# apache/arrow-go

Hardware: AMD Instinct MI355X
Metric: GB/s processed per kernel (Sum/Add/Filter/Take) vs HBM roofline (higher is better)
Workload: dtype int64+f64

## Files before the change

### arrow_go_amd/csrc/ah_common.h

```cpp
#pragma once
#include <hip/hip_runtime.h>
#include <initializer_list>
#include <type_traits>
#include <stdarg.h>
#include <stdint.h>
#include <stddef.h>
#include <stdio.h>
#include <stdlib.h>
#include <string.h>
#include "../../include/arrowhip.h"

#define AH_EXPORT extern "C" __attribute__((visibility("default")))

struct ah_filter_cache {
  bool valid;
  const uint8_t *fdata, *fvalid;
  int64_t foff, n, ntiles;
  int null_sel, tile_rows;
  void* buf;
  size_t bytes;
  int64_t* super_off;
  int* tile_local;
  int64_t* total;
};

struct ah_ctx {
  int device;
  hipStream_t stream;
  hipStream_t copy_stream;
  bool owns_stream;
  hipEvent_t ev_copy;
  hipEvent_t ev_compute;
  hipEvent_t t0, t1;
  hipEvent_t* marks;
  int n_marks;
  void* scratch;
  size_t scratch_bytes;
  void* temp;
  size_t temp_bytes;
  void* pack;
  size_t pack_bytes;
  uint64_t* pinned;
  uint64_t* dscalars;
  int num_cu;
  int tune_nt;
  int tune_blocks_per_cu;
  int opt_take_binned, opt_take_window_log2, opt_take_gather_wg, opt_take_gather_load, opt_take_gather_lds;
  int opt_groupby_keys;
  int opt_groupby_partition;
  int opt_encode_partition;
  int opt_encode_part_slots;
  int opt_encode_byte_map;
  int opt_encode_early_look;
  int opt_encode_part_min;
  int opt_hash_direct;
  int opt_hash_sum_partition;
  int opt_sort_msd;
  int opt_scan_segment_log2;
  void* expr_cache;
  int capturing;
  ah_filter_cache fcache;
  int opt_scan_onepass;
  void* scan_recs;
  size_t scan_recs_bytes;
  unsigned scan_epoch;
  int opt_groupby_seed;
  int opt_groupby_reserve;
  int opt_groupby_lean;
  int opt_filter_cache;
  int take_clustered_hint;
  int opt_take_vec;
  bool take_hint_valid, take_hint_live;
  const void* take_hint_idx; int64_t take_hint_nidx; int take_hint_kind, take_hint_near, take_hint_uses, opt_take_hint_cache;
  unsigned long long take_hint_word;
  int opt_arith_xcd_map;
  int opt_groupby_scale_guess;
  int opt_encode_unperm2_group;
  int opt_encode_resolve_wgs;
  int opt_encode_dict_compact;
  int opt_encode_table_batch;
  int opt_encode_unperm_group;
  int opt_take_vec_nt;
  unsigned long long* mailbox;
  unsigned long long mailbox_seq;
  char err[512];
};

static inline unsigned ah_stream_grid(const ah_ctx* c, int64_t work_items, int default_bpc = 8) {
  int bpc = c->tune_blocks_per_cu > 0 ? c->tune_blocks_per_cu : default_bpc;
  int64_t cap = bpc > 0 ? (int64_t)c->num_cu * bpc : ((int64_t)1 << 30);
  int64_t g = work_items < cap ? work_items : cap;
  return (unsigned)(g < 1 ? 1 : g);
}

static inline int ah_fail(ah_ctx* ctx, int code, const char* fmt, ...) __attribute__((format(printf, 3, 4)));
static inline int ah_fail(ah_ctx* ctx, int code, const char* fmt, ...) {
  if (ctx) {
    va_list ap;
    va_start(ap, fmt);
    vsnprintf(ctx->err, sizeof(ctx->err), fmt, ap);
    va_end(ap);
  }
  return code;
}

#define AH_HIP(ctx, call)                                                              \
  do {                                                                                 \
    hipError_t e__ = (call);                                                           \
    if (e__ != hipSuccess)                                                             \
      return ah_fail((ctx), AH_EHIP, "%s failed: %s (%s:%d)", #call, hipGetErrorString(e__), \
                     __FILE__, __LINE__);                                              \
  } while (0)

#define AH_ENTER_KEEP(ctx)                                             \
  do {                                                                 \
    if (!(ctx)) return AH_EINVALID;                                    \
    (ctx)->err[0] = 0;                                                 \
    AH_HIP((ctx), hipSetDevice((ctx)->device));                        \
  } while (0)

#define AH_ENTER(ctx)                                                  \
  do {                                                                 \
    AH_ENTER_KEEP(ctx);                                                \
    (ctx)->fcache.valid = false;                                       \
    (ctx)->take_hint_valid = false;                                    \
  } while (0)

static inline bool ah_take_hint_overlaps(const ah_ctx* c, const void* p, size_t nbytes) {
  if (!c->take_hint_valid || !c->take_hint_idx) return false;
  const uintptr_t a = (uintptr_t)p, b = a + nbytes, lo = (uintptr_t)c->take_hint_idx, hi = lo + (size_t)c->take_hint_nidx * (size_t)(c->take_hint_kind / 2);
  return a < hi && lo < b;
}
static inline bool ah_fcache_overlaps(const ah_ctx* c, const void* p, size_t nbytes) {
  if (!c->fcache.valid) return false;
  const uintptr_t a = (uintptr_t)p, b = a + nbytes;
  const uintptr_t lo = (uintptr_t)(c->fcache.foff >> 3), hi = (uintptr_t)((c->fcache.foff + c->fcache.n + 7) >> 3);
  for (const uint8_t* bm : {c->fcache.fdata, c->fcache.fvalid})
    if (bm && a < (uintptr_t)bm + hi && (uintptr_t)bm + lo < b) return true;
// ... 276 lines not shown
```

### arrow_go_amd/csrc/ah_ctx.hip

```cpp
#include <chrono>
#include "ah_common.h"

static const char* kVersion = "arrowhip 0.1 (gfx950)";

AH_EXPORT const char* ah_version(void) { return kVersion; }

AH_EXPORT int ah_device_count(int* n_host) {
  int n = 0;
  hipError_t e = hipGetDeviceCount(&n);
  if (n_host) *n_host = (e == hipSuccess) ? n : 0;
  return e == hipSuccess ? AH_OK : AH_EHIP;
}

static int ctx_init_common(ah_ctx* c) {
  AH_HIP(c, hipStreamCreateWithFlags(&c->copy_stream, hipStreamNonBlocking));
  AH_HIP(c, hipEventCreateWithFlags(&c->ev_copy, hipEventDisableTiming));
  AH_HIP(c, hipEventCreateWithFlags(&c->ev_compute, hipEventDisableTiming));
  AH_HIP(c, hipEventCreate(&c->t0));
  AH_HIP(c, hipEventCreate(&c->t1));
  AH_HIP(c, hipHostMalloc((void**)&c->pinned, 64 * sizeof(uint64_t), hipHostMallocDefault));
  AH_HIP(c, hipMalloc((void**)&c->dscalars, (kDsScalars + kPopcountMaxPartials) * sizeof(uint64_t)));
  AH_HIP(c, hipMemset(c->dscalars, 0, (kDsScalars + kPopcountMaxPartials) * sizeof(uint64_t)));
  AH_HIP(c, hipHostMalloc((void**)&c->mailbox, 256, hipHostMallocCoherent | hipHostMallocMapped));
  memset(c->mailbox, 0, 256);
  hipDeviceProp_t prop;
  AH_HIP(c, hipGetDeviceProperties(&prop, c->device));
  c->num_cu = prop.multiProcessorCount > 0 ? prop.multiProcessorCount : 256;
  const char* e_nt = getenv("ARROWHIP_NT");
  c->tune_nt = e_nt ? atoi(e_nt) : 1;
  const char* e_bpc = getenv("ARROWHIP_BLOCKS_PER_CU");
  c->tune_blocks_per_cu = e_bpc ? atoi(e_bpc) : 0;
  auto env_int = [](const char* name, int dflt) { const char* e = getenv(name); return e ? atoi(e) : dflt; };
  c->opt_take_binned = env_int("ARROWHIP_TAKE_BINNED", 1);
  c->opt_take_window_log2 = env_int("ARROWHIP_TAKE_WINDOW_LOG2", 22);
  c->opt_take_gather_wg = env_int("ARROWHIP_TAKE_GATHER_WG_PER_CU", 8);
  c->opt_groupby_partition = env_int("ARROWHIP_GROUPBY_PARTITION", 1);
  c->opt_groupby_keys = env_int("ARROWHIP_GROUPBY_KEYS", 1280);
  c->opt_hash_direct = env_int("ARROWHIP_HASH_DIRECT", 2);
  c->opt_hash_sum_partition = env_int("ARROWHIP_HASH_PARTITION", 1);
  c->opt_encode_partition = env_int("ARROWHIP_ENCODE_PARTITION", 1);
  c->opt_encode_part_min = env_int("ARROWHIP_ENCODE_PART_MIN", 300000);
  c->opt_encode_early_look = env_int("ARROWHIP_ENCODE_EARLY_LOOK", 1);
  c->opt_encode_byte_map = env_int("ARROWHIP_ENCODE_BYTE_MAP", 1);
  c->opt_encode_part_slots = env_int("ARROWHIP_ENCODE_PART_SLOTS", 8192);
  c->opt_sort_msd = env_int("ARROWHIP_SORT_MSD", 1);
  c->opt_scan_segment_log2 = env_int("ARROWHIP_SCAN_SEGMENT_LOG2", 0);
  c->opt_take_gather_lds = env_int("ARROWHIP_TAKE_GATHER_LDS", 1);
  c->opt_take_vec_nt = env_int("ARROWHIP_TAKE_VEC_NT", 7);
  c->opt_encode_unperm_group = env_int("ARROWHIP_ENCODE_UNPERM_GROUP", 4);
  c->opt_encode_table_batch = env_int("ARROWHIP_ENCODE_TABLE_BATCH", 1);
  c->opt_encode_dict_compact = env_int("ARROWHIP_ENCODE_DICT_COMPACT", 1);
  c->opt_encode_resolve_wgs = env_int("ARROWHIP_ENCODE_RESOLVE_WGS", 1024);
  c->opt_encode_unperm2_group = env_int("ARROWHIP_ENCODE_UNPERM2_GROUP", 4);
  c->opt_groupby_scale_guess = env_int("ARROWHIP_GROUPBY_SCALE_GUESS", 1);
  c->opt_arith_xcd_map = env_int("ARROWHIP_ARITH_XCD_MAP", 0);
  c->opt_take_vec = env_int("ARROWHIP_TAKE_VEC", 1);
  c->opt_take_gather_load = env_int("ARROWHIP_TAKE_GATHER_LOAD", 0);
  return AH_OK;
}

static int ctx_create(int device_id, void* stream, bool borrow, ah_ctx** out) {
  if (!out) return AH_EINVALID;
  *out = nullptr;
  ah_ctx* c = (ah_ctx*)calloc(1, sizeof(ah_ctx));
  if (!c) return AH_EINVALID;
  c->device = device_id;
  hipError_t e = hipSetDevice(device_id);
  if (e != hipSuccess) { free(c); return AH_EHIP; }
  if (borrow) {
    c->stream = (hipStream_t)stream;
    c->owns_stream = false;
  } else {
    e = hipStreamCreateWithFlags(&c->stream, hipStreamNonBlocking);
    if (e != hipSuccess) { free(c); return AH_EHIP; }
    c->owns_stream = true;
  }
  int rc = ctx_init_common(c);
  if (rc != AH_OK) { fprintf(stderr, "arrowhip: ctx init failed: %s\n", c->err); free(c); return rc; }
  c->opt_filter_cache = c->owns_stream ? 1 : 0;
  c->opt_take_hint_cache = c->owns_stream ? 1 : 0;
  c->opt_groupby_lean = 1;
  c->opt_scan_onepass = 1;
  c->opt_groupby_seed = 1;
  c->opt_groupby_reserve = 1;
  *out = c;
  return AH_OK;
}

AH_EXPORT int ah_ctx_create(int device_id, ah_ctx** out) { return ctx_create(device_id, nullptr, false, out); }
AH_EXPORT int ah_ctx_create_on_stream(int device_id, void* hip_stream, ah_ctx** out) {
  return ctx_create(device_id, hip_stream, true, out);
}

AH_EXPORT void ah_ctx_destroy(ah_ctx* c) {
  if (!c) return;
  (void)hipSetDevice(c->device);
  (void)hipStreamSynchronize(c->stream);
  (void)hipStreamSynchronize(c->copy_stream);
  ah_expr_cache_free(c);
  if (c->scratch) (void)hipFree(c->scratch);
  if (c->pinned) (void)hipHostFree(c->pinned);
  if (c->dscalars) (void)hipFree(c->dscalars);
  if (c->mailbox) (void)hipHostFree(c->mailbox);
  if (c->fcache.buf) (void)hipFree(c->fcache.buf);
  if (c->scan_recs) (void)hipFree(c->scan_recs);
  if (c->temp) (void)hipFree(c->temp);
  if (c->pack) (void)hipFree(c->pack);
  (void)hipEventDestroy(c->ev_copy);
  (void)hipEventDestroy(c->ev_compute);
  (void)hipEventDestroy(c->t0);
  (void)hipEventDestroy(c->t1);
  for (int i = 0; i < c->n_marks; i++) if (c->marks[i]) (void)hipEventDestroy(c->marks[i]);
  free(c->marks);
  (void)hipStreamDestroy(c->copy_stream);
  if (c->owns_stream) (void)hipStreamDestroy(c->stream);
  free(c);
}

AH_EXPORT int ah_ctx_set_option(ah_ctx* c, const char* name, int64_t value) {
  AH_ENTER(c);
  if (!name) return ah_fail(c, AH_EINVALID, "set_option: null name");
  if (!strcmp(name, "nt")) c->tune_nt = (int)value;
  else if (!strcmp(name, "blocks_per_cu")) c->tune_blocks_per_cu = (int)value;
  else if (!strcmp(name, "take_binned")) c->opt_take_binned = (int)value;
  else if (!strcmp(name, "take_window_log2")) c->opt_take_window_log2 = (int)value;
  else if (!strcmp(name, "take_gather_wg_per_cu")) c->opt_take_gather_wg = (int)value;
  else if (!strcmp(name, "take_gather_lds")) c->opt_take_gather_lds = (int)value;
  else if (!strcmp(name, "take_vec")) c->opt_take_vec = (int)value;
  else if (!strcmp(name, "take_hint_cache")) { c->opt_take_hint_cache = (int)value; c->take_hint_valid = false; }
  else if (!strcmp(name, "take_vec_nt")) c->opt_take_vec_nt = (int)value;
  else if (!strcmp(name, "encode_unperm_group")) c->opt_encode_unperm_group = (int)value;
  else if (!strcmp(name, "encode_table_batch")) c->opt_encode_table_batch = (int)value;
  else if (!strcmp(name, "encode_dict_compact")) c->opt_encode_dict_compact = (int)value;
  else if (!strcmp(name, "encode_unperm2_group")) c->opt_encode_unperm2_group = (int)value;
  else if (!strcmp(name, "encode_resolve_wgs")) c->opt_encode_resolve_wgs = value < 1 ? 1 : (int)value;
  else if (!strcmp(name, "groupby_scale_guess")) c->opt_groupby_scale_guess = (int)value;
  else if (!strcmp(name, "arith_xcd_map")) c->opt_arith_xcd_map = (int)value;
  else if (!strcmp(name, "take_gather_load")) c->opt_take_gather_load = (int)value;
  else if (!strcmp(name, "groupby_partition")) c->opt_groupby_partition = (int)value;
  else if (!strcmp(name, "groupby_keys")) c->opt_groupby_keys = (int)value;
  else if (!strcmp(name, "hash_direct")) c->opt_hash_direct = (int)value;
  else if (!strcmp(name, "hash_sum_partition")) c->opt_hash_sum_partition = (int)value;
  else if (!strcmp(name, "encode_partition")) c->opt_encode_partition = (int)value;
  else if (!strcmp(name, "encode_part_min")) c->opt_encode_part_min = (int)value;
  else if (!strcmp(name, "encode_early_look")) c->opt_encode_early_look = (int)value;
  else if (!strcmp(name, "encode_byte_map")) c->opt_encode_byte_map = (int)value;
  else if (!strcmp(name, "encode_part_slots")) c->opt_encode_part_slots = (int)value;
  else if (!strcmp(name, "sort_msd")) c->opt_sort_msd = (int)value;
  else if (!strcmp(name, "scan_onepass")) c->opt_scan_onepass = (int)value;
  else if (!strcmp(name, "groupby_lean")) c->opt_groupby_lean = (int)value;
  else if (!strcmp(name, "groupby_seed")) c->opt_groupby_seed = (int)value;
  else if (!strcmp(name, "groupby_reserve")) c->opt_groupby_reserve = (int)value;
  else if (!strcmp(name, "filter_cache")) { c->opt_filter_cache = value != 0; if (!value) c->fcache.valid = false; }
  else if (!strcmp(name, "scan_segment_log2")) c->opt_scan_segment_log2 = (int)value;
  else return ah_fail(c, AH_EINVALID, "set_option: unknown option '%s'", name);
  return AH_OK;
}

AH_EXPORT const char* ah_last_error(ah_ctx* c) { return c ? c->err : "null context"; }

namespace {
__global__ void mailbox_post_kernel(const unsigned long long* __restrict__ src, int nwords, const unsigned long long* __restrict__ src2, int nwords2,
                                    unsigned long long* mailbox, unsigned long long seq) {
  for (int i = 0; i < nwords; i++) __hip_atomic_store(&mailbox[i], src[i], __ATOMIC_RELAXED, __HIP_MEMORY_SCOPE_SYSTEM);
  for (int i = 0; i < nwords2; i++) __hip_atomic_store(&mailbox[nwords + i], src2[i], __ATOMIC_RELAXED, __HIP_MEMORY_SCOPE_SYSTEM);
  __hip_atomic_store(&mailbox[7], seq, __ATOMIC_RELEASE, __HIP_MEMORY_SCOPE_SYSTEM);
}
}
int ah_mailbox_read(ah_ctx* c, const unsigned long long* dev_words, int nwords, unsigned long long* out_host) {
  return ah_mailbox_read2(c, dev_words, nwords, nullptr, 0, out_host);
}
int ah_mailbox_begin(ah_ctx* c, unsigned long long** mb_out, unsigned long long* seq_out) {
  if (c->capturing) { c->capturing = 2; return ah_fail(c, AH_EINVALID, "this call returns a value to the host: it cannot be recorded into a graph"); }
  *mb_out = c->mailbox + 8;
  *seq_out = ++c->mailbox_seq;
  return AH_OK;
}
int ah_mailbox_wait(ah_ctx* c, unsigned long long seq, int nwords, unsigned long long* out_host) {
  if (nwords < 1 || nwords > 7) return ah_fail(c, AH_EINVALID, "mailbox_wait: 1..7 words");
  unsigned long long* mb = c->mailbox + 8;
  bool seen = false;
  const auto t0 = std::chrono::steady_clock::now();
  for (unsigned spin = 0;; spin++) {
    if (__atomic_load_n(&mb[7], __ATOMIC_ACQUIRE) == seq) { seen = true; break; }
    __builtin_ia32_pause();
    if ((spin & 1023u) == 1023u && std::chrono::steady_clock::now() - t0 > std::chrono::milliseconds(5)) break;
  }
  if (!seen) {
    AH_HIP(c, hipStreamSynchronize(c->stream));
    if (__atomic_load_n(&mb[7], __ATOMIC_ACQUIRE) != seq) return ah_fail(c, AH_EHIP, "mailbox_wait: the kernel did not report");
  }
  for (int i = 0; i < nwords; i++) out_host[i] = __atomic_load_n(&mb[i], __ATOMIC_RELAXED);
  return AH_OK;
}
int ah_mailbox_read2(ah_ctx* c, const unsigned long long* dev_words, int nwords, const unsigned long long* dev_words2, int nwords2,
                     unsigned long long* out_host) {
  if (nwords < 1 || nwords2 < 0 || nwords + nwords2 > 7) return ah_fail(c, AH_EINVALID, "mailbox_read: 1..7 words");
  if (c->capturing) { c->capturing = 2; return ah_fail(c, AH_EINVALID, "this call returns a value to the host: it cannot be recorded into a graph"); }
  unsigned long long* mb = c->mailbox + 8;
  const unsigned long long seq = ++c->mailbox_seq;
  mailbox_post_kernel<<<1, 1, 0, c->stream>>>(dev_words, nwords, dev_words2, nwords2, mb, seq);
  AH_LAUNCH_CHECK(c);
  bool seen = false;
  const auto t0 = std::chrono::steady_clock::now();
  for (unsigned spin = 0;; spin++) {
    if (__atomic_load_n(&mb[7], __ATOMIC_ACQUIRE) == seq) { seen = true; break; }
    __builtin_ia32_pause();
    if ((spin & 1023u) == 1023u && std::chrono::steady_clock::now() - t0 > std::chrono::milliseconds(5)) break;
  }
  if (!seen) {
    AH_HIP(c, hipStreamSynchronize(c->stream));
    if (__atomic_load_n(&mb[7], __ATOMIC_ACQUIRE) != seq) return ah_fail(c, AH_EHIP, "mailbox_read: the post kernel did not report");
  }
  for (int i = 0; i < nwords + nwords2; i++) out_host[i] = __atomic_load_n(&mb[i], __ATOMIC_RELAXED);
  return AH_OK;
}

int ah_scratch_reserve(ah_ctx* c, size_t nbytes, void** out) {
  if (nbytes > c->scratch_bytes) {
    AH_HIP(c, hipStreamSynchronize(c->stream));
    if (c->scratch) AH_HIP(c, hipFree(c->scratch));
    c->scratch = nullptr;
    c->scratch_bytes = 0;
    size_t want = (nbytes + ((size_t)1 << 20) - 1) & ~(((size_t)1 << 20) - 1);
// ... 295 lines not shown
```

### arrow_go_amd/csrc/ah_hash.hip

```cpp
#include "ah_common.h"
#include "ah_hashing.h"
#include "ah_bytes.h"

namespace {


struct Slot {
  unsigned long long key;
  unsigned first_row;
  unsigned id;
};


struct U64Keys {
  const unsigned long long* keys;
  static constexpr bool kLdsTable = true;
  __device__ __forceinline__ bool load(int64_t i, unsigned long long* word, uint64_t* h) const {
    const unsigned long long k = keys[i];
    *word = k;
    *h = hash_int(k);
    return k != kEmpty;
  }
  __device__ __forceinline__ bool same(unsigned long long cur, unsigned long long word, int64_t) const { return cur == word; }
};
// ... 137 lines not shown
      k[u] = 0;
      idx[u] = 0;
      if (i < hi) {
        if (ah_bit(valid, off + i)) {
          uint64_t h;
          if (!keys.load(i, &k[u], &h)) { kind[u] = 2; idx[u] = cap; }
          else { kind[u] = 1; idx[u] = h & mask; }
        } else if (encode_nulls) { kind[u] = 2; idx[u] = cap + 1; }
        else kind[u] = 3;
      }
    }
#pragma unroll
    for (int u = 0; u < kInsertRows; u++)
      if (kind[u] == 1 || kind[u] == 2) sv[u] = load_slot(&table[idx[u]]);
#pragma unroll
    for (int u = 0; u < kInsertRows; u++) {
      const int64_t i = base + (int64_t)u * kBlock;
      if (kind[u] == 0) continue;
      if (kind[u] == 3) { if (row_slot) row_slot[i] = direct_below ? 0u : kNoRow; continue; }
      uint64_t s = idx[u];
      unsigned fr = sv[u].first_row;
      unsigned id = sv[u].id;
      if (kind[u] == 1) {
        unsigned long long cur = sv[u].key;
        int probes = 0;
        for (;;) {
          if (cur == kEmpty) {
            cur = atomicCAS(&table[s].key, kEmpty, k[u]);
            if (cur == kEmpty) { fresh++; break; }
          }
          if (keys.same(cur, k[u], i)) break;
          s = (s + 1) & mask;
          if (++probes > kProbeLimit) { atomicExch(overflow, 1u); return; }
          const SlotView nx = load_slot(&table[s]);
          cur = nx.key;
          fr = nx.first_row;
          id = nx.id;
        }
      }
      if (fr < direct_below) {
        if (row_slot) row_slot[i] = id;
        continue;
      }
      if (fr > (unsigned)i) atomicMin(&table[s].first_row, (unsigned)i);
      if (row_slot) row_slot[i] = (unsigned)s | flag;
      nmiss++;
    }
  }
  if (fresh) atomicAdd(distinct, (unsigned long long)fresh);
  if (direct_below && nmiss) atomicAdd(misses, (unsigned long long)nmiss);
}

__global__ __launch_bounds__(kBlock) void mark_kernel(const Slot* __restrict__ table, uint64_t nslots,
                                                       unsigned long long* __restrict__ firsts) {
  const int64_t stride = (int64_t)gridDim.x * kBlock;
  for (uint64_t s = (uint64_t)blockIdx.x * kBlock + threadIdx.x; s < nslots; s += stride) {
    unsigned fr = table[s].first_row;
    if (fr != kNoRow) atomicOr(&firsts[fr >> 6], 1ull << (fr & 63));
  }
}


__global__ __launch_bounds__(kBlock) void assign_kernel(Slot* __restrict__ table, uint64_t cap, const unsigned long long* __restrict__ firsts,
                                                         const unsigned* __restrict__ wordprefix, const int64_t* __restrict__ tileoff,
                                                         unsigned long long* __restrict__ dict, int* __restrict__ null_id,
                                                         long long* __restrict__ first_rows) {
  const int64_t stride = (int64_t)gridDim.x * kBlock;
  const uint64_t nslots = cap + 2;
  for (uint64_t s = (uint64_t)blockIdx.x * kBlock + threadIdx.x; s < nslots; s += stride) {
    unsigned fr = table[s].first_row;
    if (fr == kNoRow) continue;
    unsigned id = rank_of_row(fr, firsts, wordprefix, tileoff);
    table[s].id = id;
    if (first_rows) first_rows[id] = (long long)fr;
    if (s == cap + 1) {
      *null_id = (int)id;
      if (dict) dict[id] = 0;
    } else if (dict) {
      dict[id] = table[s].key;
    }
  }
}

__global__ __launch_bounds__(kBlock) void emit_kernel(const Slot* __restrict__ table, int32_t* __restrict__ ids, int64_t n, int64_t direct_from) {
  constexpr int U = 4;
  const int64_t stride = (int64_t)gridDim.x * kBlock * U;
  for (int64_t base = (int64_t)blockIdx.x * kBlock * U + threadIdx.x; base < n; base += stride) {
    unsigned s[U];
    int32_t id[U];
    bool put[U];
#pragma unroll
    for (int u = 0; u < U; u++) {
      const int64_t i = base + (int64_t)u * kBlock;
      s[u] = i < n ? (unsigned)ids[i] : kNoRow;
      put[u] = i < n;
      if (i >= direct_from && s[u] != kNoRow) {
        if (s[u] & 0x80000000u) s[u] &= 0x7fffffffu; else put[u] = false;
      }
    }
#pragma unroll
    for (int u = 0; u < U; u++) id[u] = s[u] == kNoRow ? 0 : (put[u] ? (int32_t)table[s[u]].id : 0);
#pragma unroll
    for (int u = 0; u < U; u++) {
      const int64_t i = base + (int64_t)u * kBlock;
      if (put[u]) ids[i] = id[u];
    }
  }
}

constexpr unsigned kLookup = 0xFFFFFFFEu;
struct InsertSide {
  uint64_t cap;
  int encode_nulls;
  unsigned ones_id, null_id;
  __device__ __forceinline__ InsertSide(const Slot* t, uint64_t cap_, int encode_nulls_)
      : cap(cap_), encode_nulls(encode_nulls_), ones_id(t[cap_].first_row != kNoRow ? t[cap_].id : kNoRow),
        null_id(t[cap_ + 1].first_row != kNoRow ? t[cap_ + 1].id : kNoRow) {}
};

__device__ __forceinline__ bool claim_slot(unsigned long long k, Slot* __restrict__ table, uint64_t mask, int limit, unsigned* __restrict__ overflow,
                                           uint64_t* slot, unsigned* inserted) {
  uint64_t s = hash_int(k) & mask;
  int probes = 0;
  for (;;) {
    unsigned long long cur = table[s].key;
    if (cur != k && cur == kEmpty) {
      cur = atomicCAS(&table[s].key, kEmpty, k);
      if (cur == kEmpty) { (*inserted)++; cur = k; }
    }
    if (cur == k) break;
    s = (s + 1) & mask;
    if (++probes > limit) { atomicExch(overflow, 1u); return false; }
  }
  *slot = s;
  return true;
}

__device__ __forceinline__ unsigned row_without_lookup(const InsertSide& t, bool ok, unsigned long long k, uint64_t* s) {
  *s = ok ? t.cap : t.cap + 1;
  if (!ok) return t.encode_nulls ? t.null_id : 0u;
  return k == kEmpty ? t.ones_id : kLookup;
}
__device__ __forceinline__ bool miss_row(Slot* __restrict__ table, uint64_t mask, unsigned* __restrict__ overflow, unsigned long long k, int64_t i, bool probe,
                                         uint64_t s, unsigned* fresh, unsigned* nmiss, unsigned* r) {
  if (probe && !claim_slot(k, table, mask, kProbeLimit, overflow, &s, fresh)) return false;
  if (table[s].first_row > (unsigned)i) atomicMin(&table[s].first_row, (unsigned)i);
  *r = 0x80000000u | (unsigned)s;
  (*nmiss)++;
  return true;
}

constexpr int kSmallSlots = 8192;
constexpr int kSmallKeys = 4096;
constexpr int kSmallBlock = 1024;
constexpr int kSmallRows = 8;

__global__ __launch_bounds__(kBlock) void small_build_kernel(const Slot* __restrict__ table, uint64_t cap,
                                                              unsigned long long* __restrict__ skeys, unsigned* __restrict__ sids) {
  const int64_t stride = (int64_t)gridDim.x * kBlock;
  for (uint64_t s = (uint64_t)blockIdx.x * kBlock + threadIdx.x; s < cap; s += stride) {
    if (table[s].first_row == kNoRow) continue;
    const unsigned long long k = table[s].key;
    unsigned j = (unsigned)hash_int(k) & (kSmallSlots - 1);
    while (atomicCAS(&skeys[j], kEmpty, k) != kEmpty) j = (j + 1) & (kSmallSlots - 1);
    sids[j] = table[s].id;
  }
// ... 74 lines not shown
  unsigned long long key;
  unsigned id;
  unsigned pad;
};
__global__ __launch_bounds__(kBlock) void compact_build_kernel(const Slot* __restrict__ table, uint64_t cap, CSlot* __restrict__ ctab, uint64_t cmask) {
  const int64_t stride = (int64_t)gridDim.x * kBlock;
  for (uint64_t s = (uint64_t)blockIdx.x * kBlock + threadIdx.x; s < cap; s += stride) {
    const SlotView v = load_slot(&table[s]);
    if (v.first_row == kNoRow) continue;
    uint64_t j = hash_int(v.key) & cmask;
    while (atomicCAS(&ctab[j].key, kEmpty, v.key) != kEmpty) j = (j + 1) & cmask;
    ctab[j].id = v.id;
  }
}

constexpr int kCompactRows = 8;
__global__ __launch_bounds__(kBlock) void insert_compact_kernel(const unsigned long long* __restrict__ keys, const uint8_t* __restrict__ valid,
                                                                 int64_t off, int64_t lo, int64_t hi, int encode_nulls, Slot* __restrict__ table,
                                                                 uint64_t cap, const CSlot* __restrict__ ctab, uint64_t cmask,
                                                                 unsigned* __restrict__ out_ids, unsigned long long* __restrict__ distinct,
                                                                 unsigned* __restrict__ overflow, unsigned long long* __restrict__ misses) {
  const InsertSide side(table, cap, encode_nulls);
  const uint64_t mask = cap - 1;
  const int64_t stride = (int64_t)gridDim.x * kBlock * kCompactRows;
  unsigned fresh = 0, nmiss = 0;
  for (int64_t base = lo + (int64_t)blockIdx.x * kBlock * kCompactRows + threadIdx.x; base < hi; base += stride) {
    unsigned long long k[kCompactRows];
    bool ok[kCompactRows];
    uint4 cs[kCompactRows];
#pragma unroll
    for (int u = 0; u < kCompactRows; u++) {
      const int64_t i = base + (int64_t)u * kBlock;
      ok[u] = i < hi && ah_bit(valid, off + i);
      k[u] = ok[u] ? __builtin_nontemporal_load(&keys[i]) : 0ull;
    }
#pragma unroll
    for (int u = 0; u < kCompactRows; u++) cs[u] = *reinterpret_cast<const uint4*>(&ctab[hash_int(k[u]) & cmask]);
#pragma unroll
    for (int u = 0; u < kCompactRows; u++) {
      const int64_t i = base + (int64_t)u * kBlock;
      if (i >= hi) break;
      uint64_t s;
      bool probe = false;
      unsigned r = row_without_lookup(side, ok[u], k[u], &s);
      if (r == kLookup) {
        r = kNoRow;
        uint64_t j = hash_int(k[u]) & cmask;
        uint4 c = cs[u];
        for (;;) {
          const unsigned long long ck = ((unsigned long long)c.y << 32) | c.x;
          if (ck == k[u]) { r = c.z; break; }
          if (ck == kEmpty) { probe = true; break; }
          j = (j + 1) & cmask;
          c = *reinterpret_cast<const uint4*>(&ctab[j]);
        }
      }
      if (r == kNoRow && !miss_row(table, mask, overflow, k[u], i, probe, s, &fresh, &nmiss, &r)) return;
      if (out_ids) __builtin_nontemporal_store(r, &out_ids[i]);
    }
  }
  if (fresh) atomicAdd(distinct, (unsigned long long)fresh);
  if (nmiss) atomicAdd(misses, (unsigned long long)nmiss);
}

static uint64_t next_pow2_u64(uint64_t x) {
  uint64_t p = 1;
  while (p < x) p <<= 1;
  return p;
}

static double estimate_distinct(double d0, double p, double n) {
  const double r = d0 / p;
  if (r >= 0.999) return n;
  double lo = 1e-9, hi = 64.0;
  for (int it = 0; it < 60; it++) {
    const double mid = 0.5 * (lo + hi);
    if ((1.0 - exp(-mid)) / mid > r) lo = mid; else hi = mid;
  }
  const double C = p / (0.5 * (lo + hi));
  const double d = C * (1.0 - exp(-n / C));
  return d < n ? d : n;
}

struct EncodeResult {
  int64_t ndict;
  int32_t null_id;
};

template <typename K>
int encode_core(ah_ctx* c, const K keys, const uint8_t* valid, int64_t off, int64_t n, int encode_nulls,
                int32_t* out_ids, uint64_t* out_dict, EncodeResult* res, int64_t* out_first_rows = nullptr, bool allow_partitioned = true) {
  res->ndict = 0;
  res->null_id = -1;
  if (n == 0) return AH_OK;
  auto try_partitioned = [&](int lp, bool* done, int slots2 = 4096) -> int {
    *done = false;
    if constexpr (K::kLdsTable) {
      int used = 0;
      int64_t nd = 0;
      int32_t nid = -1;
      int prc = lp <= 10 ? ah_encode_partitioned_try(c, (const uint64_t*)keys.keys, valid, off, n, encode_nulls, lp, c->opt_encode_part_slots == 4096 ? 4096 : 8192, out_ids, out_dict, out_first_rows, &nd, &nid, &used)
                         : ah_encode_partitioned2_try(c, (const uint64_t*)keys.keys, valid, off, n, encode_nulls, lp, slots2, out_ids, out_dict, out_first_rows, &nd, &nid, &used);
      if (prc != AH_OK) return prc;
      if (used) { res->ndict = nd; res->null_id = nid; *done = true; }
    }
    return AH_OK;
  };
  if (K::kLdsTable && allow_partitioned && c->opt_encode_partition >= 3) {
    bool done;
    int prc = try_partitioned(c->opt_encode_partition > 13 ? 13 : c->opt_encode_partition, &done);
    if (prc != AH_OK || done) return prc;
  }
  if (n > ((int64_t)1 << 30)) return ah_fail(c, AH_ENOTIMPL, "hash: more than 2^30 rows per call");
  auto decide_after_look = [&](double d16, bool overflowed, bool* undecided, bool* done, bool* attempted) -> int {
    const double hi = (double)((int64_t)1 << 16);
    *done = false;
    *attempted = false;
    const double est = estimate_distinct(d16, hi, (double)n);
    *undecided = !overflowed && d16 >= 0.999 * hi;
    if (overflowed || est < (double)c->opt_encode_part_min || est > 8192.0 * 4400.0) return AH_OK;
    int lp = 8;
    const double kpp1 = c->opt_encode_part_slots == 4096 ? 2200.0 : 4400.0;
    while (lp < 10 && est / (double)(1 << lp) > kpp1) lp++;
    int slots2 = 4096;
    if (est / (double)(1 << lp) > kpp1) {
      lp = 11;
      while (lp < 13 && est / (double)(1 << lp) > 2200.0) lp++;
      if (est / (double)(1 << lp) > 2600.0) slots2 = 8192;
    }
    *attempted = true;
    return try_partitioned(lp, done, slots2);
  };
  bool looked = false, look_undecided = false;
  if constexpr (K::kLdsTable) if (allow_partitioned && c->opt_encode_partition == 1 && n >= ((int64_t)1 << 24) && c->opt_encode_early_look) {
    uint64_t d16 = 0;
    int lrc = ah_encode_first_look(c, (const uint64_t*)keys.keys, valid, off, (int64_t)1 << 16, &d16);
    if (lrc != AH_OK) return lrc;
    bool done = false, attempted = false;
    lrc = decide_after_look((double)d16, false, &look_undecided, &done, &attempted);
    if (lrc != AH_OK || done) return lrc;
    looked = true;
  }
  const int64_t nwords = ah_ceil_div(n, 64);
  const int64_t ntiles = ah_ceil_div(nwords, 32);
  const uint64_t cap_max = next_pow2_u64((uint64_t)n * 2 < 64 ? 64 : (uint64_t)n * 2);
  uint64_t cap = cap_max < ((uint64_t)1 << 22) ? cap_max : ((uint64_t)1 << 22);
  unsigned long long* distinct = (unsigned long long*)&c->dscalars[4];
  unsigned* overflow = (unsigned*)&c->dscalars[5];
  unsigned long long* total = (unsigned long long*)&c->dscalars[6];
  int* null_id = (int*)&c->dscalars[7];
  unsigned long long* misses = (unsigned long long*)&c->dscalars[8];
  const int direct_path = c->opt_hash_direct;
  bool resized = false;
  for (;;) {
    size_t table_bytes = (size_t)(cap + 2) * sizeof(Slot);
    size_t firsts_bytes = (size_t)nwords * 8;
    size_t wp_bytes = ((size_t)nwords * 4 + 7) & ~(size_t)7;
    size_t tc_bytes = ((size_t)ntiles * 4 + 7) & ~(size_t)7;
    size_t to_bytes = (size_t)ntiles * 8;
    void* scratch;
    const size_t small_bytes = (size_t)kSmallSlots * 12;
    const size_t compact_bytes = K::kLdsTable ? (size_t)(cap / 2) * sizeof(CSlot) : 0;
    int rc = ah_scratch_reserve(c, table_bytes + firsts_bytes + wp_bytes + tc_bytes + to_bytes + small_bytes + compact_bytes + 64, &scratch);
    if (rc != AH_OK) return rc;
    Slot* table = (Slot*)scratch;
    unsigned long long* firsts = (unsigned long long*)((uint8_t*)scratch + table_bytes);
    unsigned* wordprefix = (unsigned*)((uint8_t*)firsts + firsts_bytes);
    int* tilecnt = (int*)((uint8_t*)wordprefix + wp_bytes);
    int64_t* tileoff = (int64_t*)((uint8_t*)tilecnt + tc_bytes);
    unsigned long long* skeys = (unsigned long long*)((uint8_t*)tileoff + to_bytes);
    unsigned* sids = (unsigned*)(skeys + kSmallSlots);
    CSlot* ctab = (CSlot*)(((uintptr_t)(sids + kSmallSlots) + 63) & ~(uintptr_t)63);

    AH_HIP(c, hipMemsetAsync(table, 0xFF, table_bytes, c->stream));
    AH_HIP(c, hipMemsetAsync(&c->dscalars[4], 0, 3 * sizeof(uint64_t), c->stream));
    AH_HIP(c, hipMemsetAsync(null_id, 0xFF, sizeof(uint64_t), c->stream));
    const int64_t prefix = n < ((int64_t)1 << 21) ? n : ((int64_t)1 << 21);
    unsigned grid = ah_stream_grid(c, ah_ceil_div(n, (int64_t)kBlock * kInsertRows));
    bool part_undecided = false;
    auto restore_slot_numbers = [&](int64_t rows) -> int {
      if (!out_ids || rows <= 0) return AH_OK;
      insert_kernel<K><<<ah_stream_grid(c, ah_ceil_div(rows, (int64_t)kBlock * kInsertRows)), kBlock, 0, c->stream>>>(
          keys, valid, off, 0, rows, encode_nulls, table, cap, (unsigned*)out_ids, 0u, 0u, distinct, overflow, misses);
      AH_LAUNCH_CHECK(c);
      return AH_OK;
    };
    {
      int64_t lo = 0;
      for (int64_t hi : {(int64_t)1 << 12, (int64_t)1 << 16, prefix}) {
        if (hi > prefix) hi = prefix;
        if (hi <= lo) continue;
        unsigned g = ah_stream_grid(c, ah_ceil_div(hi - lo, (int64_t)kBlock * kInsertRows));
        insert_kernel<K><<<g, kBlock, 0, c->stream>>>(keys, valid, off, lo, hi, encode_nulls, table, cap,
                                                   (unsigned*)out_ids, 0u, 0u, distinct, overflow, misses);
        AH_LAUNCH_CHECK(c);
        lo = hi;
        if (K::kLdsTable && allow_partitioned && c->opt_encode_partition == 1 && !resized && !looked && hi == ((int64_t)1 << 16) && n >= ((int64_t)1 << 22)) {
          unsigned long long look[2];
          if ((rc = ah_mailbox_read(c, (const unsigned long long*)&c->dscalars[4], 2, look)) != AH_OK) return rc;
          c->pinned[0] = look[0]; c->pinned[1] = look[1];
          bool done, attempted;
          int prc = decide_after_look((double)look[0], (unsigned)look[1] != 0, &part_undecided, &done, &attempted);
          if (prc != AH_OK || done) return prc;
          if (attempted && (prc = restore_slot_numbers(hi)) != AH_OK) return prc;
        }
      }
    }
    if (looked && !resized) part_undecided = look_undecided;
    bool restart = false, small = false, direct = false, compact = false;
    uint64_t d0 = 0;
    if (prefix < n && cap < cap_max) {
      if ((rc = ah_mailbox_read(c, (const unsigned long long*)&c->dscalars[4], 2, (unsigned long long*)c->pinned)) != AH_OK) return rc;
      d0 = *(volatile uint64_t*)&c->pinned[0];
      bool ovf = *(volatile unsigned*)&c->pinned[1] != 0;
      if (part_undecided && !ovf) {
        const double est = estimate_distinct((double)d0, (double)prefix, (double)n);
        if (est <= 8192.0 * 4400.0) {
          bool done;
          int prc = try_partitioned(13, &done, est / 8192.0 > 2600.0 ? 8192 : 4096);
          if (prc != AH_OK || done) return prc;
          if ((prc = restore_slot_numbers(prefix)) != AH_OK) return prc;
        }
      }
      if (ovf || d0 > cap / 4) {
        uint64_t want = next_pow2_u64((uint64_t)(estimate_distinct((double)d0, (double)prefix, (double)n) * 3.0) + 64);
        if (want < cap * 4) want = cap * 4;
        cap = want < cap_max ? want : cap_max;
        restart = true;
        resized = true;
      }
      direct = !restart && !ovf && !resized && direct_path;
      small = K::kLdsTable && direct && d0 <= (uint64_t)kSmallKeys && direct_path > 1;
      compact = K::kLdsTable && direct && !small && direct_path > 1 && direct_path != 3;
    }
    if (restart) continue;
    auto rank_slots = [&](int64_t rows) -> int {
      const int64_t nw = ah_ceil_div(rows, 64), nt = rank_tiles(nw);
      AH_HIP(c, hipMemsetAsync(firsts, 0, (size_t)nw * 8, c->stream));
      mark_kernel<<<ah_stream_grid(c, ah_ceil_div((int64_t)cap + 2, kBlock)), kBlock, 0, c->stream>>>(table, cap + 2, firsts);
      AH_LAUNCH_CHECK(c);
      word_prefix_kernel<<<(unsigned)ah_ceil_div(nw, kBlock), kBlock, 0, c->stream>>>(firsts, nw, wordprefix, tilecnt);
      AH_LAUNCH_CHECK(c);
      scan_kernel<<<1, 1024, 0, c->stream>>>(tilecnt, nt, tileoff, total);
      AH_LAUNCH_CHECK(c);
      assign_kernel<<<ah_stream_grid(c, ah_ceil_div((int64_t)cap + 2, kBlock)), kBlock, 0, c->stream>>>(
          table, cap, firsts, wordprefix, tileoff, (unsigned long long*)out_dict, null_id, (long long*)out_first_rows);
      AH_LAUNCH_CHECK(c);
      return AH_OK;
    };
    int64_t direct_from = n;
    bool ranked = false;
    if (direct) {
      if ((rc = rank_slots(prefix)) != AH_OK) return rc;
      AH_HIP(c, hipMemsetAsync(misses, 0, 8, c->stream));
      direct_from = prefix;
      int64_t lo = prefix;
      if constexpr (K::kLdsTable) if (small) {
        AH_HIP(c, hipMemsetAsync(skeys, 0xFF, (size_t)kSmallSlots * 8, c->stream));
        small_build_kernel<<<ah_stream_grid(c, ah_ceil_div((int64_t)cap, kBlock)), kBlock, 0, c->stream>>>(table, cap, skeys, sids);
        AH_LAUNCH_CHECK(c);
        const int64_t probe_end = n - prefix > ((int64_t)1 << 23) ? prefix + ((int64_t)1 << 22) : n;
        const unsigned sgrid = (unsigned)c->num_cu;
        insert_small_kernel<<<sgrid, kSmallBlock, 0, c->stream>>>(keys.keys, valid, off, prefix, probe_end, encode_nulls,
                                                                  table, cap, skeys, sids, (unsigned*)out_ids, distinct, overflow, misses);
        AH_LAUNCH_CHECK(c);
        lo = probe_end;
        if (probe_end < n) {
          if ((rc = ah_mailbox_read(c, misses, 1, (unsigned long long*)c->pinned)) != AH_OK) return rc;
          if (*(volatile uint64_t*)c->pinned * 8 < (uint64_t)(probe_end - prefix)) {
            insert_small_kernel<<<sgrid, kSmallBlock, 0, c->stream>>>(keys.keys, valid, off, probe_end, n, encode_nulls,
                                                                      table, cap, skeys, sids, (unsigned*)out_ids, distinct, overflow, misses);
            AH_LAUNCH_CHECK(c);
            lo = n;
          }
        }
      }
      if constexpr (K::kLdsTable) if (compact && lo < n) {
        const uint64_t ccap = next_pow2_u64(d0 * 2 < 64 ? 64 : d0 * 2);
        AH_HIP(c, hipMemsetAsync(ctab, 0xFF, (size_t)ccap * sizeof(CSlot), c->stream));
        compact_build_kernel<<<ah_stream_grid(c, ah_ceil_div((int64_t)cap, kBlock)), kBlock, 0, c->stream>>>(table, cap, ctab, ccap - 1);
        AH_LAUNCH_CHECK(c);
        const int64_t seg_lo = lo, probe_end = n - lo > ((int64_t)1 << 23) ? lo + ((int64_t)1 << 22) : n;
        insert_compact_kernel<<<ah_stream_grid(c, ah_ceil_div(probe_end - lo, (int64_t)kBlock * kCompactRows)), kBlock, 0, c->stream>>>(
            keys.keys, valid, off, lo, probe_end, encode_nulls, table, cap, ctab, ccap - 1, (unsigned*)out_ids, distinct, overflow, misses);
        AH_LAUNCH_CHECK(c);
        lo = probe_end;
        if (probe_end < n) {
          if ((rc = ah_mailbox_read(c, misses, 1, (unsigned long long*)c->pinned)) != AH_OK) return rc;
          if (*(volatile uint64_t*)c->pinned * 64 < (uint64_t)(probe_end - seg_lo)) {
            insert_compact_kernel<<<ah_stream_grid(c, ah_ceil_div(n - lo, (int64_t)kBlock * kCompactRows)), kBlock, 0, c->stream>>>(
                keys.keys, valid, off, lo, n, encode_nulls, table, cap, ctab, ccap - 1, (unsigned*)out_ids, distinct, overflow, misses);
            AH_LAUNCH_CHECK(c);
            lo = n;
          }
        }
      }
      if (lo < n) {
        insert_kernel<K><<<grid, kBlock, 0, c->stream>>>(keys, valid, off, lo, n, encode_nulls, table, cap,
                                                      (unsigned*)out_ids, 0x80000000u, (unsigned)prefix, distinct, overflow, misses);
        AH_LAUNCH_CHECK(c);
      }
      {
        unsigned long long w5[5];
        if ((rc = ah_mailbox_read(c, (const unsigned long long*)&c->dscalars[4], 5, w5)) != AH_OK) return rc;
        c->pinned[0] = w5[4]; c->pinned[1] = w5[1];
      }
      ranked = *(volatile uint64_t*)&c->pinned[0] == 0 && *(volatile unsigned*)&c->pinned[1] == 0;
      *(volatile uint64_t*)c->pinned = *(volatile uint64_t*)&c->pinned[1];
    } else {
      if (prefix < n) {
        insert_kernel<K><<<grid, kBlock, 0, c->stream>>>(keys, valid, off, prefix, n, encode_nulls, table, cap,
                                                      (unsigned*)out_ids, 0u, 0u, distinct, overflow, misses);
        AH_LAUNCH_CHECK(c);
      }
      if ((rc = ah_mailbox_read(c, (const unsigned long long*)overflow, 1, (unsigned long long*)c->pinned)) != AH_OK) return rc;
    }
    if (*(volatile unsigned*)c->pinned) {
      if (cap >= cap_max) return ah_fail(c, AH_EINVALID, "hash: table overflow at maximum capacity (internal error)");
      cap = cap * 16 < cap_max ? cap * 16 : cap_max;
      resized = true;
      continue;
    }
    if (!ranked && (rc = rank_slots(n)) != AH_OK) return rc;
    if (out_ids) {
      const int64_t rows = ranked ? prefix : n;
      emit_kernel<<<ah_stream_grid(c, ah_ceil_div(rows, (int64_t)kBlock * 4)), kBlock, 0, c->stream>>>(table, out_ids, rows, direct_from);
      AH_LAUNCH_CHECK(c);
    }
    if ((rc = ah_mailbox_read(c, (const unsigned long long*)&c->dscalars[6], 2, (unsigned long long*)c->pinned)) != AH_OK) return rc;
    res->ndict = (int64_t) * (volatile uint64_t*)&c->pinned[0];
    res->null_id = *(volatile int32_t*)&c->pinned[1];
    return AH_OK;
  }
}

}

int ah_encode_u64_groups(ah_ctx* c, const uint64_t* keys, const uint8_t* kvalid, int64_t koff, int64_t n, int32_t* ids, uint64_t* out_keys,
                         int64_t* out_first_rows, int64_t* out_ngroups, int32_t* out_null_group) {
  EncodeResult res;
  int rc = encode_core(c, U64Keys{(const unsigned long long*)keys}, kvalid, koff, n, 1, ids, out_keys, &res, out_first_rows, false);
  if (rc != AH_OK) return rc;
  *out_ngroups = res.ndict;
  *out_null_group = res.null_id;
  return AH_OK;
}

int ah_encode_u64_first_seen(ah_ctx* c, const uint64_t* keys, const uint8_t* valid, int64_t off, int64_t n, int32_t* ids, int64_t* out_first_rows,
                             int64_t* out_ngroups) {
  EncodeResult res;
  int rc = encode_core(c, U64Keys{(const unsigned long long*)keys}, valid, off, n, 1, ids, nullptr, &res, out_first_rows);
  if (rc != AH_OK) return rc;
  *out_ngroups = res.ndict;
  return AH_OK;
}

int ah_encode_tuple_first_seen(ah_ctx* c, int ncols, const ah_group_key* keys, int64_t n, int32_t* ids, int64_t* out_first_rows, int64_t* out_ngroups) {
  KeyCol cols[8];
  for (int j = 0; j < 8; j++) {
    cols[j] = KeyCol{nullptr, nullptr, nullptr, 0, kColNone, 0};
    if (j >= ncols) continue;
    const ah_group_key& k = keys[j];
    if (k.offset_width == 4) cols[j] = KeyCol{(const int32_t*)k.offsets + k.off, k.data, k.valid, k.off, kColVar4, 0};
    else if (k.offset_width == 8) cols[j] = KeyCol{(const long long*)k.offsets + k.off, k.data, k.valid, k.off, kColVar8, 0};
    else if (k.bits) cols[j] = KeyCol{nullptr, k.data, k.valid, k.off, kColBits, 0};
    else cols[j] = KeyCol{nullptr, k.data + k.off * (int64_t)k.byte_width, k.valid, k.off, kColFixed, k.byte_width};
  }
  EncodeResult res;
  int rc;
  auto run = [&](auto keys_of) { rc = encode_core(c, keys_of, nullptr, 0, n, 1, ids, nullptr, &res, out_first_rows); };
  if (ncols <= 2) { TupleKeys<2> t; for (int j = 0; j < 2; j++) t.col[j] = cols[j]; run(t); }
  else if (ncols <= 4) { TupleKeys<4> t; for (int j = 0; j < 4; j++) t.col[j] = cols[j]; run(t); }
  else { TupleKeys<8> t; for (int j = 0; j < 8; j++) t.col[j] = cols[j]; run(t); }
  if (rc != AH_OK) return rc;
  *out_ngroups = res.ndict;
  return AH_OK;
}

static int encode_finish(ah_ctx* c, const EncodeResult& res, const uint8_t* valid, int64_t off, int64_t n, int encode_nulls, uint8_t* out_ids_valid,
                         int64_t* out_ndict_host, int32_t* out_null_id_host) {
  if (out_ids_valid) {
    AH_HIP(c, hipMemsetAsync(out_ids_valid, 0, (size_t)((n + 7) / 8), c->stream));
    int rc = valid && !encode_nulls ? ah_copy_bitmap(c, valid, off, n, out_ids_valid, 0, 0) : ah_set_bits_to(c, out_ids_valid, 0, n, 1);
    if (rc != AH_OK) return rc;
    AH_HIP(c, hipStreamSynchronize(c->stream));
  }
  if (out_ndict_host) *out_ndict_host = res.ndict;
  if (out_null_id_host) *out_null_id_host = res.null_id;
  return AH_OK;
}

AH_EXPORT int ah_hash_binary_encode(ah_ctx* c, int offset_width, const void* offsets, const uint8_t* data, const uint8_t* valid, int64_t off,
                                    int64_t n, int encode_nulls, int32_t* out_ids, uint8_t* out_ids_valid, int64_t* out_first_rows,
                                    int64_t* out_ndict_host, int32_t* out_null_id_host) {
  AH_ENTER(c);
  if (n < 0 || off < 0) return ah_fail(c, AH_EINVALID, "hash: negative length/offset");
  if (offset_width != 4 && offset_width != 8) return ah_fail(c, AH_EINVALID, "hash: offset width must be 4 or 8");
  if (out_ndict_host) *out_ndict_host = 0;
// ... 67 lines not shown
```

Baseline: 6381.

## Size hash table from early distinct-count look and add single-block small rank kernel

Adds a table-sizing option, on by default, that uses the early distinct-count sample to start the hash table at a capacity proportional to the observed distinct keys. When the sample looks saturated, the prefix shrinks to the look rows. For small tables it replaces the mark/scan/rank pipeline with one workgroup that bitonic-sorts occupied slots by first row in LDS and can also build the small probe table. This cuts memset and rank-pass cost on low-cardinality encodes. The price is more control-flow complexity and extra resize/restart risk if the estimate is wrong.

Result: no change. 6429 (median of 3 runs) (+0.8%).

```diff
diff --git a/arrow_go_amd/csrc/ah_common.h b/arrow_go_amd/csrc/ah_common.h
--- a/arrow_go_amd/csrc/ah_common.h
+++ b/arrow_go_amd/csrc/ah_common.h
@@ -54,6 +54,7 @@
   int opt_encode_early_look;
   int opt_encode_part_min;
   int opt_hash_direct;
+  int opt_hash_table_sizing;
   int opt_hash_sum_partition;
   int opt_sort_msd;
   int opt_scan_segment_log2;
diff --git a/arrow_go_amd/csrc/ah_ctx.hip b/arrow_go_amd/csrc/ah_ctx.hip
--- a/arrow_go_amd/csrc/ah_ctx.hip
+++ b/arrow_go_amd/csrc/ah_ctx.hip
@@ -37,6 +37,7 @@
   c->opt_groupby_partition = env_int("ARROWHIP_GROUPBY_PARTITION", 1);
   c->opt_groupby_keys = env_int("ARROWHIP_GROUPBY_KEYS", 1280);
   c->opt_hash_direct = env_int("ARROWHIP_HASH_DIRECT", 2);
+  c->opt_hash_table_sizing = env_int("ARROWHIP_HASH_TABLE_SIZING", 1);
   c->opt_hash_sum_partition = env_int("ARROWHIP_HASH_PARTITION", 1);
   c->opt_encode_partition = env_int("ARROWHIP_ENCODE_PARTITION", 1);
   c->opt_encode_part_min = env_int("ARROWHIP_ENCODE_PART_MIN", 300000);
@@ -140,6 +141,7 @@
   else if (!strcmp(name, "groupby_partition")) c->opt_groupby_partition = (int)value;
   else if (!strcmp(name, "groupby_keys")) c->opt_groupby_keys = (int)value;
   else if (!strcmp(name, "hash_direct")) c->opt_hash_direct = (int)value;
+  else if (!strcmp(name, "hash_table_sizing")) c->opt_hash_table_sizing = (int)value;
   else if (!strcmp(name, "hash_sum_partition")) c->opt_hash_sum_partition = (int)value;
   else if (!strcmp(name, "encode_partition")) c->opt_encode_partition = (int)value;
   else if (!strcmp(name, "encode_part_min")) c->opt_encode_part_min = (int)value;
diff --git a/arrow_go_amd/csrc/ah_hash.hip b/arrow_go_amd/csrc/ah_hash.hip
--- a/arrow_go_amd/csrc/ah_hash.hip
+++ b/arrow_go_amd/csrc/ah_hash.hip
@@ -243,6 +243,74 @@
   }
 }
 
+constexpr int kRankSmallMax = 2048;
+constexpr uint64_t kRankSmallCap = (uint64_t)1 << 15;
+constexpr int kRankSmallBlock = 1024;
+__global__ __launch_bounds__(kRankSmallBlock) void rank_small_kernel(Slot* __restrict__ table, uint64_t cap, unsigned long long* __restrict__ dict,
+                                                                      int* __restrict__ null_id, long long* __restrict__ first_rows,
+                                                                      unsigned long long* __restrict__ total, unsigned long long* __restrict__ skeys,
+                                                                      unsigned* __restrict__ sids, unsigned nsmall) {
+  __shared__ unsigned long long s_pair[kRankSmallMax];
+  __shared__ unsigned s_used;
+  const unsigned tid = threadIdx.x;
+  for (unsigned j = tid; j < (unsigned)kRankSmallMax; j += kRankSmallBlock) s_pair[j] = ~0ull;
+  if (tid == 0) s_used = 0;
+  if (skeys) {
+    for (unsigned j = tid; j < nsmall; j += kRankSmallBlock) skeys[j] = kEmpty;
+    __threadfence();
+  }
+  __syncthreads();
+  constexpr int U = 8;
+  const uint64_t nslots = cap + 2;
+  for (uint64_t base = tid; base < nslots; base += (uint64_t)kRankSmallBlock * U) {
+    unsigned fr[U];
+#pragma unroll
+    for (int u = 0; u < U; u++) {
+      const uint64_t s = base + (uint64_t)u * kRankSmallBlock;
+      fr[u] = s < nslots ? table[s].first_row : kNoRow;
+    }
+#pragma unroll
+    for (int u = 0; u < U; u++) {
+      if (fr[u] == kNoRow) continue;
+      const unsigned p = atomicAdd(&s_used, 1u);
+      if (p < (unsigned)kRankSmallMax) s_pair[p] = ((unsigned long long)fr[u] << 32) | (unsigned long long)(base + (uint64_t)u * kRankSmallBlock);
+    }
+  }
+  __syncthreads();
+  const unsigned m = s_used < (unsigned)kRankSmallMax ? s_used : (unsigned)kRankSmallMax;
+  unsigned M = 2;
+  while (M < m) M <<= 1;
+  for (unsigned k = 2; k <= M; k <<= 1) {
+    for (unsigned j = k >> 1; j > 0; j >>= 1) {
+      for (unsigned t = tid; t < (M >> 1); t += kRankSmallBlock) {
+        const unsigned i = ((t & ~(j - 1)) << 1) | (t & (j - 1)), l = i | j;
+        const unsigned long long a = s_pair[i], b = s_pair[l];
+        if ((a > b) == ((i & k) == 0)) { s_pair[i] = b; s_pair[l] = a; }
+      }
+      __syncthreads();
+    }
+  }
+  for (unsigned p = tid; p < m; p += kRankSmallBlock) {
+    const unsigned long long pr = s_pair[p];
+    const uint64_t s = (unsigned)pr;
+    table[s].id = p;
+    if (first_rows) first_rows[p] = (long long)(pr >> 32);
+    if (s == cap + 1) {
+      *null_id = (int)p;
+      if (dict) dict[p] = 0;
+    } else {
+      const unsigned long long key = table[s].key;
+      if (dict) dict[p] = key;
+      if (skeys && s < cap) {
+        unsigned j = (unsigned)hash_int(key) & (nsmall - 1);
+        while (atomicCAS(&skeys[j], kEmpty, key) != kEmpty) j = (j + 1) & (nsmall - 1);
+        sids[j] = p;
+      }
+    }
+  }
+  if (tid == 0) *total = (unsigned long long)m;
+}
+
 __global__ __launch_bounds__(kBlock) void emit_kernel(const Slot* __restrict__ table, int32_t* __restrict__ ids, int64_t n, int64_t direct_from) {
   constexpr int U = 4;
   const int64_t stride = (int64_t)gridDim.x * kBlock * U;
@@ -483,6 +551,18 @@
   return d < n ? d : n;
 }
 
+static bool look_saturated(double d, double p, double n) {
+  if (d * 64.0 <= p) return true;
+  return estimate_distinct(d, p, n) - d < 0.01;
+}
+
+constexpr uint64_t kCapFloor = (uint64_t)1 << 12, kCapFirstStages = (uint64_t)1 << 18, kCapStartMax = (uint64_t)1 << 22;
+constexpr int64_t kSizeByReadRows = (int64_t)1 << 18;
+static uint64_t start_capacity(double slots, uint64_t cap_limit) {
+  const uint64_t want = next_pow2_u64(slots < (double)kCapStartMax ? (uint64_t)slots + 1 : kCapStartMax);
+  return want < kCapFloor ? (kCapFloor < cap_limit ? kCapFloor : cap_limit) : (want < cap_limit ? want : cap_limit);
+}
+
 struct EncodeResult {
   int64_t ndict;
   int32_t null_id;
@@ -533,6 +613,7 @@
     return try_partitioned(lp, done, slots2);
   };
   bool looked = false, look_undecided = false;
+  double look_d16 = 0;
   if constexpr (K::kLdsTable) if (allow_partitioned && c->opt_encode_partition == 1 && n >= ((int64_t)1 << 24) && c->opt_encode_early_look) {
     uint64_t d16 = 0;
     int lrc = ah_encode_first_look(c, (const uint64_t*)keys.keys, valid, off, (int64_t)1 << 16, &d16);
@@ -541,11 +622,24 @@
     lrc = decide_after_look((double)d16, false, &look_undecided, &done, &attempted);
     if (lrc != AH_OK || done) return lrc;
     looked = true;
+    look_d16 = (double)d16;
   }
   const int64_t nwords = ah_ceil_div(n, 64);
   const int64_t ntiles = ah_ceil_div(nwords, 32);
   const uint64_t cap_max = next_pow2_u64((uint64_t)n * 2 < 64 ? 64 : (uint64_t)n * 2);
-  uint64_t cap = cap_max < ((uint64_t)1 << 22) ? cap_max : ((uint64_t)1 << 22);
+  const uint64_t cap_limit = cap_max < kCapStartMax ? cap_max : kCapStartMax;
+  const bool sizing = c->opt_hash_table_sizing != 0;
+  const int64_t look_rows = (int64_t)1 << 16;
+  int64_t prefix = n < ((int64_t)1 << 21) ? n : ((int64_t)1 << 21);
+  uint64_t cap = cap_limit;
+  int64_t counted = -1;
+  bool size_by_read = false;
+  if (sizing && looked) {
+    if (look_saturated(look_d16, (double)look_rows, (double)n)) { prefix = look_rows; counted = (int64_t)look_d16; cap = start_capacity(4.5 * look_d16, cap_limit); }
+  } else if (c->opt_hash_table_sizing >= 2 && n > kSizeByReadRows) {
+    cap = kCapFirstStages;
+    size_by_read = true;
+  }
   unsigned long long* distinct = (unsigned long long*)&c->dscalars[4];
   unsigned* overflow = (unsigned*)&c->dscalars[5];
   unsigned long long* total = (unsigned long long*)&c->dscalars[6];
@@ -576,7 +670,6 @@
     AH_HIP(c, hipMemsetAsync(table, 0xFF, table_bytes, c->stream));
     AH_HIP(c, hipMemsetAsync(&c->dscalars[4], 0, 3 * sizeof(uint64_t), c->stream));
     AH_HIP(c, hipMemsetAsync(null_id, 0xFF, sizeof(uint64_t), c->stream));
-    const int64_t prefix = n < ((int64_t)1 << 21) ? n : ((int64_t)1 << 21);
     unsigned grid = ah_stream_grid(c, ah_ceil_div(n, (int64_t)kBlock * kInsertRows));
     bool part_undecided = false;
     auto restore_slot_numbers = [&](int64_t rows) -> int {
@@ -586,6 +679,7 @@
       AH_LAUNCH_CHECK(c);
       return AH_OK;
     };
+    bool resize_now = false;
     {
       int64_t lo = 0;
       for (int64_t hi : {(int64_t)1 << 12, (int64_t)1 << 16, prefix}) {
@@ -596,24 +690,45 @@
                                                    (unsigned*)out_ids, 0u, 0u, distinct, overflow, misses);
         AH_LAUNCH_CHECK(c);
         lo = hi;
-        if (K::kLdsTable && allow_partitioned && c->opt_encode_partition == 1 && !resized && !looked && hi == ((int64_t)1 << 16) && n >= ((int64_t)1 << 22)) {
+        const bool part_look = K::kLdsTable && allow_partitioned && c->opt_encode_partition == 1 && n >= ((int64_t)1 << 22);
+        if ((part_look || size_by_read) && !resized && !looked && hi == look_rows) {
           unsigned long long look[2];
           if ((rc = ah_mailbox_read(c, (const unsigned long long*)&c->dscalars[4], 2, look)) != AH_OK) return rc;
           c->pinned[0] = look[0]; c->pinned[1] = look[1];
-          bool done, attempted;
-          int prc = decide_after_look((double)look[0], (unsigned)look[1] != 0, &part_undecided, &done, &attempted);
-          if (prc != AH_OK || done) return prc;
-          if (attempted && (prc = restore_slot_numbers(hi)) != AH_OK) return prc;
+          if (part_look) {
+            bool done, attempted;
+            int prc = decide_after_look((double)look[0], (unsigned)look[1] != 0, &part_undecided, &done, &attempted);
+            if (prc != AH_OK || done) return prc;
+            if (attempted && !size_by_read && (prc = restore_slot_numbers(hi)) != AH_OK) return prc;
+          }
+          if (size_by_read) {
+            size_by_read = false;
+            looked = true;
+            look_undecided = part_undecided;
+            const bool saturated = (unsigned)look[1] == 0 && look_saturated((double)look[0], (double)look_rows, (double)n);
+            if (saturated) { prefix = look_rows; counted = (int64_t)look[0]; }
+            cap = saturated ? start_capacity(4.5 * (double)look[0], cap_limit) : cap_limit;
+            resize_now = true;
+            break;
+          }
         }
       }
     }
+    if (resize_now) continue;
     if (looked && !resized) part_undecided = look_undecided;
     bool restart = false, small = false, direct = false, compact = false;
     uint64_t d0 = 0;
+    uint64_t dseen = ~(uint64_t)0;
     if (prefix < n && cap < cap_max) {
-      if ((rc = ah_mailbox_read(c, (const unsigned long long*)&c->dscalars[4], 2, (unsigned long long*)c->pinned)) != AH_OK) return rc;
-      d0 = *(volatile uint64_t*)&c->pinned[0];
-      bool ovf = *(volatile unsigned*)&c->pinned[1] != 0;
+      bool ovf = false;
+      if (counted >= 0 && !resized) {
+        d0 = (uint64_t)counted;
+      } else {
+        if ((rc = ah_mailbox_read(c, (const unsigned long long*)&c->dscalars[4], 2, (unsigned long long*)c->pinned)) != AH_OK) return rc;
+        d0 = *(volatile uint64_t*)&c->pinned[0];
+        ovf = *(volatile unsigned*)&c->pinned[1] != 0;
+      }
+      dseen = d0;
       if (part_undecided && !ovf) {
         const double est = estimate_distinct((double)d0, (double)prefix, (double)n);
         if (est <= 8192.0 * 4400.0) {
@@ -635,7 +750,15 @@
       compact = K::kLdsTable && direct && !small && direct_path > 1 && direct_path != 3;
     }
     if (restart) continue;
-    auto rank_slots = [&](int64_t rows) -> int {
+    bool small_built = false;
+    auto rank_slots = [&](int64_t rows, bool build_small = false) -> int {
+      if (sizing && cap <= kRankSmallCap && dseen <= (uint64_t)(kRankSmallMax - 2)) {
+        rank_small_kernel<<<1, kRankSmallBlock, 0, c->stream>>>(table, cap, (unsigned long long*)out_dict, null_id, (long long*)out_first_rows, total,
+                                                                build_small ? skeys : nullptr, sids, (unsigned)kSmallSlots);
+        AH_LAUNCH_CHECK(c);
+        small_built = build_small;
+        return AH_OK;
+      }
       const int64_t nw = ah_ceil_div(rows, 64), nt = rank_tiles(nw);
       AH_HIP(c, hipMemsetAsync(firsts, 0, (size_t)nw * 8, c->stream));
       mark_kernel<<<ah_stream_grid(c, ah_ceil_div((int64_t)cap + 2, kBlock)), kBlock, 0, c->stream>>>(table, cap + 2, firsts);
@@ -652,14 +775,16 @@
     int64_t direct_from = n;
     bool ranked = false;
     if (direct) {
-      if ((rc = rank_slots(prefix)) != AH_OK) return rc;
+      if ((rc = rank_slots(prefix, small)) != AH_OK) return rc;
       AH_HIP(c, hipMemsetAsync(misses, 0, 8, c->stream));
       direct_from = prefix;
       int64_t lo = prefix;
       if constexpr (K::kLdsTable) if (small) {
-        AH_HIP(c, hipMemsetAsync(skeys, 0xFF, (size_t)kSmallSlots * 8, c->stream));
-        small_build_kernel<<<ah_stream_grid(c, ah_ceil_div((int64_t)cap, kBlock)), kBlock, 0, c->stream>>>(table, cap, skeys, sids);
-        AH_LAUNCH_CHECK(c);
+        if (!small_built) {
+          AH_HIP(c, hipMemsetAsync(skeys, 0xFF, (size_t)kSmallSlots * 8, c->stream));
+          small_build_kernel<<<ah_stream_grid(c, ah_ceil_div((int64_t)cap, kBlock)), kBlock, 0, c->stream>>>(table, cap, skeys, sids);
+          AH_LAUNCH_CHECK(c);
+        }
         const int64_t probe_end = n - prefix > ((int64_t)1 << 23) ? prefix + ((int64_t)1 << 22) : n;
         const unsigned sgrid = (unsigned)c->num_cu;
         insert_small_kernel<<<sgrid, kSmallBlock, 0, c->stream>>>(keys.keys, valid, off, prefix, probe_end, encode_nulls,
@@ -705,6 +830,7 @@
         unsigned long long w5[5];
         if ((rc = ah_mailbox_read(c, (const unsigned long long*)&c->dscalars[4], 5, w5)) != AH_OK) return rc;
         c->pinned[0] = w5[4]; c->pinned[1] = w5[1];
+        dseen = w5[0];
       }
       ranked = *(volatile uint64_t*)&c->pinned[0] == 0 && *(volatile unsigned*)&c->pinned[1] == 0;
       *(volatile uint64_t*)c->pinned = *(volatile uint64_t*)&c->pinned[1];
@@ -714,7 +840,12 @@
                                                       (unsigned*)out_ids, 0u, 0u, distinct, overflow, misses);
         AH_LAUNCH_CHECK(c);
       }
-      if ((rc = ah_mailbox_read(c, (const unsigned long long*)overflow, 1, (unsigned long long*)c->pinned)) != AH_OK) return rc;
+      {
+        unsigned long long w2[2];
+        if ((rc = ah_mailbox_read(c, (const unsigned long long*)&c->dscalars[4], 2, w2)) != AH_OK) return rc;
+        dseen = w2[0];
+        c->pinned[0] = w2[1];
+      }
     }
     if (*(volatile unsigned*)c->pinned) {
       if (cap >= cap_max) return ah_fail(c, AH_EINVALID, "hash: table overflow at maximum capacity (internal error)");
```
